# marcemq/crowdmod-ddpm-4D

Hardware: AMD Instinct MI355X
Metric: denoise-steps/sec (UNet fwd + sampler update) at ATC [B,4,T,H,W] (higher is better)
Workload: dtype f32; 1 GPU; config/ATC.yml sampling on the 12x36 grid, fp32 arithmetic (fp32 matrix instructions; fp32 products built from f16 two-way splits -- three v_mfma_f32_32x32x16_f16 cross terms, fp32 accumulate, same error against the reference as round 3's six-term bf16 form -- in the Winograd / quarter-resolution / last-conv layers, whose input is GroupNorm + SiLU output, and in the upsample layers, whose raw inpu; channels=4, past_len=5, future_len=3, global_batch=64, parallelism=batch-shard x1 (2 stream lanes of 32 chains per rank)

## Files before the change

crowdmod-ddpm-4d_amd/csrc/cm_attn_block.hip:

```cpp
#include "cm_kernels.h"

#include <algorithm>
#include <atomic>

namespace cm {

typedef float f32x4 __attribute__((ext_vector_type(4)));

constexpr int ATT_NT = 768;
constexpr int ATT_KS = 3;

template <int D>
__global__ __launch_bounds__(ATT_NT) void attn_head_kernel(const AttnBlockArgs a) {
  constexpr int NT = ATT_NT, NW = NT / 64;
  constexpr int KD = D < 16 ? 16 : D;
  constexpr int DS = KD + 4;
  constexpr int NBQ = (D + 15) / 16;
  constexpr int NBT = 3 * NBQ;
  constexpr int PARTS = D / 8;
  constexpr int E = 4 * D;
  constexpr int XS = E + 8;
  constexpr int Q4 = E >> 2;
  constexpr int RL = NT / Q4;
  extern __shared__ __attribute__((aligned(16))) float sm[];
  const int S = a.S;
  float *Xs = sm;
  float *Wi = Xs + (size_t)S * XS;
  float *Wo = Wi + (size_t)NBT * 16 * XS;
  float *Qs = Wo + (size_t)E * DS;
  float *Ks = Qs + (size_t)S * DS;
  float *Vs = Ks + (size_t)S * DS;
  float *bi = Vs + (size_t)S * DS;
  float *red = bi + NBT * 16;
  const int h = blockIdx.x, b = blockIdx.y, tid = threadIdx.x;
  const int lane = tid & 63, wave = __builtin_amdgcn_readfirstlane(tid >> 6);
  const int r16 = lane & 15, kq = lane >> 4;

  const int q4 = tid % Q4, rl = tid / Q4;
  const float *xb = a.x + (size_t)b * S * E;
  constexpr int UX = 3;
  constexpr int NWI = (NBT * 16 + RL - 1) / RL;
  constexpr int NWO = (E * (KD / 4) + NT - 1) / NT;
  f32x4 vx[UX], vwi[NWI], vwo[NWO];
#pragma unroll
  for (int u = 0; u < UX; ++u) vx[u] = *reinterpret_cast<const f32x4 *>(xb + (size_t)min(rl + u * RL, S - 1) * E + 4 * q4);
#pragma unroll
  for (int u = 0; u < NWI; ++u) {
    const int wr = min(rl + u * RL, NBT * 16 - 1);
    const int which = wr / (NBQ * 16), c = min(wr % (NBQ * 16), D - 1);
    vwi[u] = *reinterpret_cast<const f32x4 *>(a.w_in + (size_t)(which * E + h * D + c) * E + 4 * q4);
  }
#pragma unroll
  for (int u = 0; u < NWO; ++u) {
    const int i = min(tid + u * NT, E * (KD / 4) - 1);
    const int n = i / (KD / 4), c4 = min(i % (KD / 4), D / 4 - 1);
    vwo[u] = *reinterpret_cast<const f32x4 *>(a.w_out + (size_t)n * E + h * D + 4 * c4);
  }
  const f32x4 ga = *reinterpret_cast<const f32x4 *>(a.gamma + 4 * q4);
  const f32x4 be = *reinterpret_cast<const f32x4 *>(a.beta + 4 * q4);
  float bval = 0.f;
  {
    const int tb = min(tid, NBT * 16 - 1);
    const int which = tb / (NBQ * 16), c = min(tb % (NBQ * 16), D - 1);
    bval = a.b_in[which * E + h * D + c];
  }
  float s1 = 0.f;
#pragma unroll
  for (int u = 0; u < UX; ++u) {
    const int row = rl + u * RL;
    if (row < S) {
      *reinterpret_cast<f32x4 *>(Xs + row * XS + 4 * q4) = vx[u];
      s1 += (vx[u][0] + vx[u][1]) + (vx[u][2] + vx[u][3]);
    }
  }
#pragma unroll
  for (int u = 0; u < NWI; ++u) {
    const int wr = rl + u * RL;
    if (wr < NBT * 16) *reinterpret_cast<f32x4 *>(Wi + wr * XS + 4 * q4) = vwi[u];
  }
#pragma unroll
  for (int u = 0; u < NWO; ++u) {
    const int i = tid + u * NT;
    if (i < E * (KD / 4)) {
      const int n = i / (KD / 4), c4 = i % (KD / 4);
      *reinterpret_cast<f32x4 *>(Wo + n * DS + 4 * c4) = (4 * c4 < D) ? vwo[u] : f32x4{0.f, 0.f, 0.f, 0.f};
    }
  }
  if (tid < NBT * 16) bi[tid] = bval;
  for (int row0 = UX * RL; row0 < S; row0 += UX * RL) {
#pragma unroll
    for (int u = 0; u < UX; ++u) vx[u] = *reinterpret_cast<const f32x4 *>(xb + (size_t)min(row0 + rl + u * RL, S - 1) * E + 4 * q4);
#pragma unroll
    for (int u = 0; u < UX; ++u) {
      const int row = row0 + rl + u * RL;
      if (row < S) {
        *reinterpret_cast<f32x4 *>(Xs + row * XS + 4 * q4) = vx[u];
        s1 += (vx[u][0] + vx[u][1]) + (vx[u][2] + vx[u][3]);
      }
    }
  }

  constexpr int QPG = Q4 / 8;
  const int grp = q4 / QPG;
  auto group_sum = [&](float v) -> float {
#pragma unroll
    for (int mk = 1; mk < QPG; mk <<= 1) v += __shfl_xor(v, mk);
    __syncthreads();
    if ((q4 & (QPG - 1)) == 0) red[rl * 8 + grp] = v;
    __syncthreads();
    if (tid < 8) {
      float t = 0.f;
      for (int r = 0; r < RL; ++r) t += red[r * 8 + tid];
      red[RL * 8 + tid] = t;
    }
    __syncthreads();
    return red[RL * 8 + grp];
  };
  const float cnt = (float)(E / 8) * (float)S;
  const float mean = group_sum(s1) / cnt;
  float s2 = 0.f;
  for (int row = rl; row < S; row += RL) {
    const f32x4 v = *reinterpret_cast<const f32x4 *>(Xs + row * XS + 4 * q4);
    const float d0 = v[0] - mean, d1 = v[1] - mean, d2 = v[2] - mean, d3 = v[3] - mean;
    s2 += (d0 * d0 + d1 * d1) + (d2 * d2 + d3 * d3);
  }
  const float rstd = rsqrtf(group_sum(s2) / cnt + a.eps);
  {
    const f32x4 sc = ga * rstd;
    const f32x4 sh = be - sc * mean;
    for (int row = rl; row < S; row += RL) {
      f32x4 *p = reinterpret_cast<f32x4 *>(Xs + row * XS + 4 * q4);
      *p = *p * sc + sh;
    }
  }
  __syncthreads();

  const int nmb = (S + 15) >> 4;
  constexpr int nj = E >> 4;
  const float qscale = rsqrtf((float)D);
  for (int item = wave; item < nmb * NBT; item += NW) {
    const int mb = item / NBT, nb = item - mb * NBT;
    const int arow = min(mb * 16 + r16, S - 1);
    const float *ap = Xs + arow * XS + 4 * kq;
    const float *bp = Wi + (nb * 16 + r16) * XS + 4 * kq;
    f32x4 af[nj], bf[nj];
#pragma unroll
    for (int j = 0; j < nj; ++j) {
      af[j] = *reinterpret_cast<const f32x4 *>(ap + 16 * j);
      bf[j] = *reinterpret_cast<const f32x4 *>(bp + 16 * j);
    }
    f32x4 acc = {0.f, 0.f, 0.f, 0.f};
#pragma unroll
    for (int j = 0; j < nj; ++j)
#pragma unroll
      for (int jj = 0; jj < 4; ++jj) acc = __builtin_amdgcn_mfma_f32_16x16x4f32(af[j][jj], bf[j][jj], acc, 0, 0, 0);
    const int which = nb / NBQ, c = (nb % NBQ) * 16 + r16;
    float *dst = which == 0 ? Qs : (which == 1 ? Ks : Vs);
    const float bias = bi[nb * 16 + r16];
#pragma unroll
    for (int reg = 0; reg < 4; ++reg) {
      const int row = mb * 16 + 4 * kq + reg;
      float v = acc[reg] + bias;
      if (which == 0) v *= qscale;
      if (c >= D) v = 0.f;
      if (row < S) dst[row * DS + c] = v;
    }
  }
  __syncthreads();

  {
    constexpr int LPR = PARTS * ATT_KS;
    constexpr int ROWS = NT / LPR;
    float *mrg = Xs;
    const int part = tid % PARTS, ksl = (tid / PARTS) % ATT_KS, prow = tid / LPR;
    const int kper = (S + ATT_KS - 1) / ATT_KS;
    const int k0 = ksl * kper, k1 = min(S, k0 + kper);
    for (int row0 = 0; row0 < S; row0 += ROWS) {
      const int row = row0 + prow;
      const int rowc = row < S ? row : S - 1;
      const f32x4 q0 = *reinterpret_cast<const f32x4 *>(Qs + rowc * DS + 8 * part);
      const f32x4 q1 = *reinterpret_cast<const f32x4 *>(Qs + rowc * DS + 8 * part + 4);
      f32x4 o0 = {0.f, 0.f, 0.f, 0.f}, o1 = {0.f, 0.f, 0.f, 0.f};
      float mx = -3.0e38f, l = 0.f;
      for (int j = k0; j < k1; ++j) {
        const f32x4 kv0 = *reinterpret_cast<const f32x4 *>(Ks + j * DS + 8 * part);
        const f32x4 kv1 = *reinterpret_cast<const f32x4 *>(Ks + j * DS + 8 * part + 4);
        float sa = q0[0] * kv0[0], sb = q1[0] * kv1[0];
        sa = fmaf(q0[1], kv0[1], sa); sb = fmaf(q1[1], kv1[1], sb);
        sa = fmaf(q0[2], kv0[2], sa); sb = fmaf(q1[2], kv1[2], sb);
        sa = fmaf(q0[3], kv0[3], sa); sb = fmaf(q1[3], kv1[3], sb);
        float sc = sa + sb;
#pragma unroll
        for (int m = 1; m < PARTS; m <<= 1) sc += __shfl_xor(sc, m);
        const f32x4 v0 = *reinterpret_cast<const f32x4 *>(Vs + j * DS + 8 * part);
        const f32x4 v1 = *reinterpret_cast<const f32x4 *>(Vs + j * DS + 8 * part + 4);
        if (sc > mx) {
          const float corr = __expf(mx - sc);
          l *= corr;
          o0 *= corr;
          o1 *= corr;
          mx = sc;
        }
        const float p = __expf(sc - mx);
        l += p;
        o0 += v0 * p;
        o1 += v1 * p;
      }
      __syncthreads();
      if (row < S) {
        float *mp = mrg + ((prow * ATT_KS + ksl) * PARTS + part) * 12;
        mp[0] = mx; mp[1] = l;
        *reinterpret_cast<f32x4 *>(mp + 4) = o0;
        *reinterpret_cast<f32x4 *>(mp + 8) = o1;
      }
      __syncthreads();
      if (ksl == 0 && row < S) {
        float M = -3.0e38f;
#pragma unroll
        for (int s2i = 0; s2i < ATT_KS; ++s2i) M = fmaxf(M, mrg[((prow * ATT_KS + s2i) * PARTS + part) * 12]);
        float L = 0.f;
        f32x4 O0 = {0.f, 0.f, 0.f, 0.f}, O1 = {0.f, 0.f, 0.f, 0.f};
#pragma unroll
        for (int s2i = 0; s2i < ATT_KS; ++s2i) {
          const float *mp = mrg + ((prow * ATT_KS + s2i) * PARTS + part) * 12;
          const float w = (mp[1] > 0.f) ? __expf(mp[0] - M) : 0.f;
          L += mp[1] * w;
          O0 += *reinterpret_cast<const f32x4 *>(mp + 4) * w;
          O1 += *reinterpret_cast<const f32x4 *>(mp + 8) * w;
        }
        const float inv = 1.0f / L;
        *reinterpret_cast<f32x4 *>(Qs + row * DS + 8 * part) = O0 * inv;
        *reinterpret_cast<f32x4 *>(Qs + row * DS + 8 * part + 4) = O1 * inv;
      }
      __syncthreads();
    }
  }

  {
    constexpr int NJ = KD / 16;
    constexpr int nbe = E >> 4;
    float *pout = a.part + ((size_t)h * a.B + b) * (size_t)S * E;
    for (int item = wave; item < nmb * nbe; item += NW) {
      const int mb = item / nbe, nb = item - mb * nbe;
      const int arow = min(mb * 16 + r16, S - 1);
      f32x4 af[NJ], bf[NJ];
#pragma unroll
      for (int j = 0; j < NJ; ++j) {
        af[j] = *reinterpret_cast<const f32x4 *>(Qs + arow * DS + 16 * j + 4 * kq);
        bf[j] = *reinterpret_cast<const f32x4 *>(Wo + (nb * 16 + r16) * DS + 16 * j + 4 * kq);
      }
      f32x4 acc = {0.f, 0.f, 0.f, 0.f};
#pragma unroll
      for (int j = 0; j < NJ; ++j)
#pragma unroll
        for (int jj = 0; jj < 4; ++jj) acc = __builtin_amdgcn_mfma_f32_16x16x4f32(af[j][jj], bf[j][jj], acc, 0, 0, 0);
      const int n = nb * 16 + r16;
#pragma unroll
      for (int reg = 0; reg < 4; ++reg) {
        const int row = mb * 16 + 4 * kq + reg;
        if (row < S) pout[(size_t)row * E + n] = acc[reg];
      }
    }
  }
}

size_t attn_block_lds_bytes(int S, int E, int heads) {
  const int D = E / heads, KD = D < 16 ? 16 : D, NBT = 3 * ((D + 15) / 16);
  return ((size_t)S * (E + 8) + (size_t)NBT * 16 * (E + 8) + (size_t)E * (KD + 4) + (size_t)3 * S * (KD + 4) + (size_t)NBT * 16 +
          (size_t)(ATT_NT / (E / 4)) * 8 + 8) * sizeof(float);
}

bool attn_block_ok(int S, int E, int heads, int groups) {
  if (heads != 4 || E % heads) return false;
  const int D = E / heads;
  if (D != 8 && D != 16 && D != 32) return false;
  if (groups != 8 || E % (4 * groups)) return false;
  return S >= 1 && attn_block_lds_bytes(S, E, heads) <= 160 * 1024;
}

hipError_t launch_attn_block(const AttnBlockArgs &a, hipStream_t st) {
  if (!attn_block_ok(a.S, a.E, a.heads, a.groups)) return hipErrorInvalidValue;
  const int D = a.E / a.heads;
  const size_t smem = attn_block_lds_bytes(a.S, a.E, a.heads);
#define CM_ATTNB(DD)                                                                                        \
  if (D == DD) {                                                                                            \
    static bool attr_set[64] = {false};                                                                     \
    int dev = 0;                                                                                            \
    (void)hipGetDevice(&dev);                                                                               \
    if (!attr_set[dev & 63]) {                                                                              \
      hipError_t e = hipFuncSetAttribute(reinterpret_cast<const void *>(attn_head_kernel<DD>),              \
                                         hipFuncAttributeMaxDynamicSharedMemorySize, 160 * 1024);           \
      if (e != hipSuccess) return e;                                                                        \
      attr_set[dev & 63] = true;                                                                            \
    }                                                                                                       \
    hipLaunchKernelGGL((attn_head_kernel<DD>), dim3(a.heads, a.B), dim3(ATT_NT), smem, st, a);                 \
    return hipGetLastError();                                                                               \
  }
  CM_ATTNB(8) CM_ATTNB(16) CM_ATTNB(32)
#undef CM_ATTNB
  return hipErrorInvalidValue;
}


typedef _Float16 f16x8a __attribute__((ext_vector_type(8)));
typedef unsigned u32x4a __attribute__((ext_vector_type(4)));

constexpr int AS_NT = 1024, AS_E = 128, AS_D = 32, AS_SMAX = 64;
constexpr int AS_HS = AS_E + 8;
constexpr int AS_QS = AS_E + 4;
constexpr int AS_RED = 512;

size_t attn_sample_lds_bytes() {
  return (size_t)2 * AS_SMAX * AS_HS * sizeof(_Float16) + ((size_t)3 * AS_SMAX * AS_QS + AS_RED) * sizeof(float);
}

bool attn_sample_ok(int S, int E, int heads, int groups) { return E == AS_E && heads == 4 && groups == 8 && S >= 1 && S <= AS_SMAX; }

__device__ __forceinline__ float as_range_scale(float m, float *inv) {
  const unsigned e = (__float_as_uint(m) >> 23) & 255u;
  int se = 267 - (int)e;
  se = se < 32 ? 32 : (se > 222 ? 222 : se);
  if (!(m > 0.f) || e == 255u) se = 127;
  *inv = __uint_as_float((unsigned)(254 - se) << 23);
  return __uint_as_float((unsigned)se << 23);
}

__global__ __launch_bounds__(AS_NT) void attn_sample_kernel(const AttnSampleArgs a) {
  constexpr int E = AS_E, D = AS_D, HS = AS_HS, QS = AS_QS, NT = AS_NT;
  extern __shared__ __attribute__((aligned(16))) unsigned char smraw[];
  _Float16 *XH = reinterpret_cast<_Float16 *>(smraw);
  _Float16 *XM = XH + AS_SMAX * HS;
  float *Qs = reinterpret_cast<float *>(XM + AS_SMAX * HS);
  float *Ks = Qs + AS_SMAX * QS;
  float *Vs = Ks + AS_SMAX * QS;
  float *red = Vs + AS_SMAX * QS;
  const int S = a.S, b = blockIdx.x, tid = threadIdx.x;
  const int lane = tid & 63, wave = __builtin_amdgcn_readfirstlane(tid >> 6);
  const int r16 = lane & 15, g4 = lane >> 4;
  const int nrb = (S + 15) >> 4;

  const int q4 = tid & 31, rl = tid >> 5;
  const float *xb = a.x + (size_t)b * S * E;
  f32x4 vx[2];
#pragma unroll
  for (int u = 0; u < 2; ++u) vx[u] = *reinterpret_cast<const f32x4 *>(xb + (size_t)min(rl + 32 * u, S - 1) * E + 4 * q4);
  const f32x4 ga = *reinterpret_cast<const f32x4 *>(a.gamma + 4 * q4);
  const f32x4 be = *reinterpret_cast<const f32x4 *>(a.beta + 4 * q4);
  const int cb0 = 3 * (wave >> 1), rbp = wave & 1;
  const u32x4a *wing = reinterpret_cast<const u32x4a *>(a.win_h2);
  u32x4a wf[3][4][2];
  float bias[3];
#pragma unroll
  for (int ci = 0; ci < 2; ++ci) {
#pragma unroll
    for (int ks = 0; ks < 4; ++ks)
#pragma unroll
      for (int t = 0; t < 2; ++t) wf[ci][ks][t] = wing[(((size_t)(cb0 + ci) * 4 + ks) * 2 + t) * 64 + lane];
  }
#pragma unroll
  for (int ci = 0; ci < 3; ++ci) bias[ci] = a.b_in[(cb0 + ci) * 16 + r16];

  const int grp = q4 >> 2;
  auto group_sum = [&](float v, float *slot) -> float {
    v += __shfl_xor(v, 1);
    v += __shfl_xor(v, 2);
    v += __shfl_xor(v, 32);
    if ((lane & 35) == 0) slot[wave * 8 + grp] = v;
    __syncthreads();
    float t = 0.f;
#pragma unroll
    for (int w = 0; w < NT / 64; ++w) t += slot[w * 8 + grp];
    return t;
  };
  float s1 = 0.f;
#pragma unroll
  for (int u = 0; u < 2; ++u)
    if (rl + 32 * u < S) s1 += (vx[u][0] + vx[u][1]) + (vx[u][2] + vx[u][3]);
  const float cnt = (float)(E / 8) * (float)S;
  const float mean = group_sum(s1, red) / cnt;
  float s2 = 0.f;
#pragma unroll
  for (int u = 0; u < 2; ++u)
    if (rl + 32 * u < S) {
      const float d0 = vx[u][0] - mean, d1 = vx[u][1] - mean, d2 = vx[u][2] - mean, d3 = vx[u][3] - mean;
      s2 += (d0 * d0 + d1 * d1) + (d2 * d2 + d3 * d3);
    }
  const float rstd = rsqrtf(group_sum(s2, red + 128) / cnt + a.eps);

  f32x4 xn[2];
  float amax = 0.f;
  {
    const f32x4 sc = ga * rstd;
    const f32x4 sh = be - sc * mean;
#pragma unroll
    for (int u = 0; u < 2; ++u) {
      xn[u] = vx[u] * sc + sh;
      if (rl + 32 * u < S) amax = fmaxf(amax, fmaxf(fmaxf(fabsf(xn[u][0]), fabsf(xn[u][1])), fmaxf(fabsf(xn[u][2]), fabsf(xn[u][3]))));
      else xn[u] = f32x4{0.f, 0.f, 0.f, 0.f};
    }
  }
  auto sample_max = [&](float v, float *slot) -> float {
#pragma unroll
    for (int off = 32; off >= 1; off >>= 1) v = fmaxf(v, __shfl_xor(v, off));
    if (lane == 0) slot[wave] = v;
    __syncthreads();
    float m = slot[0];
#pragma unroll
    for (int w = 1; w < NT / 64; ++w) m = fmaxf(m, slot[w]);
    return m;
  };
  float isa;
  const float sa = as_range_scale(sample_max(amax, red + 272), &isa);
#pragma unroll
  for (int u = 0; u < 2; ++u) {
    cm_u32x2_t t3[3];
    cm_split2_f16(xn[u] * sa, t3);
    const int row = rl + 32 * u;
    *reinterpret_cast<cm_u32x2_t *>(XH + row * HS + 4 * q4) = t3[0];
    *reinterpret_cast<cm_u32x2_t *>(XM + row * HS + 4 * q4) = t3[1];
  }
  __syncthreads();

  {
    const float osc = a.in_oscale * isa, qscale = rsqrtf((float)D);
#pragma unroll
    for (int ci = 0; ci < 3; ++ci) {
      const int cb = cb0 + ci;
      const int which = cb >> 3, c = (cb & 7) * 16 + r16;
      float *dst = which == 0 ? Qs : (which == 1 ? Ks : Vs);
      for (int rb = rbp; rb < nrb; rb += 2) {
        const _Float16 *ah = XH + (rb * 16 + r16) * HS + 8 * g4, *am = XM + (rb * 16 + r16) * HS + 8 * g4;
        f32x4 acc = {0.f, 0.f, 0.f, 0.f};
#pragma unroll
        for (int ks = 0; ks < 4; ++ks) {
          const f16x8a xh = *reinterpret_cast<const f16x8a *>(ah + 32 * ks), xm = *reinterpret_cast<const f16x8a *>(am + 32 * ks);
          const f16x8a wh = __builtin_bit_cast(f16x8a, wf[ci][ks][0]), wm = __builtin_bit_cast(f16x8a, wf[ci][ks][1]);
          acc = __builtin_amdgcn_mfma_f32_16x16x32_f16(xh, wm, acc, 0, 0, 0);
          acc = __builtin_amdgcn_mfma_f32_16x16x32_f16(xm, wh, acc, 0, 0, 0);
          acc = __builtin_amdgcn_mfma_f32_16x16x32_f16(xh, wh, acc, 0, 0, 0);
        }
#pragma unroll
        for (int reg = 0; reg < 4; ++reg) {
          float v = acc[reg] * osc + bias[ci];
          if (which == 0) v *= qscale;
          dst[(rb * 16 + 4 * g4 + reg) * QS + c] = v;
        }
      }
      if (ci == 0) {
#pragma unroll
        for (int ks = 0; ks < 4; ++ks)
#pragma unroll
          for (int t = 0; t < 2; ++t) wf[2][ks][t] = wing[(((size_t)(cb0 + 2) * 4 + ks) * 2 + t) * 64 + lane];
      }
    }
  }
  const u32x4a *woutg = reinterpret_cast<const u32x4a *>(a.wout_h2);
  const f32x4 bo = *reinterpret_cast<const f32x4 *>(a.b_out + 4 * q4);
#pragma unroll
  for (int u = 0; u < 2; ++u)
    vx[u] = *reinterpret_cast<const f32x4 *>(xb + (size_t)min(rl + 32 * u, S - 1) * E + 4 * q4);
#pragma unroll
  for (int ks = 0; ks < 4; ++ks)
#pragma unroll
    for (int t = 0; t < 2; ++t) wf[0][ks][t] = woutg[(((size_t)(wave >> 1) * 4 + ks) * 2 + t) * 64 + lane];
  __syncthreads();

  const int h = wave >> 2, qb = wave & 3;
  f32x4 oT[2] = {{0.f, 0.f, 0.f, 0.f}, {0.f, 0.f, 0.f, 0.f}};
  float omax = 0.f;
  const bool qvalid = qb * 16 + r16 < S;
  if (qb < nrb) {
    const float *qp = Qs + (qb * 16 + r16) * QS + h * D + 8 * g4;
    const f32x4 q0 = *reinterpret_cast<const f32x4 *>(qp), q1 = *reinterpret_cast<const f32x4 *>(qp + 4);
    f32x4 sc[4];
    float mx = -3.0e38f;
#pragma unroll
    for (int kb = 0; kb < 4; ++kb) {
      sc[kb] = f32x4{-3.0e38f, -3.0e38f, -3.0e38f, -3.0e38f};
      if (kb < nrb) {
        const float *kp = Ks + (kb * 16 + r16) * QS + h * D + 8 * g4;
        const f32x4 k0 = *reinterpret_cast<const f32x4 *>(kp), k1 = *reinterpret_cast<const f32x4 *>(kp + 4);
        f32x4 acc = {0.f, 0.f, 0.f, 0.f};
#pragma unroll
        for (int j = 0; j < 4; ++j) acc = __builtin_amdgcn_mfma_f32_16x16x4f32(k0[j], q0[j], acc, 0, 0, 0);
#pragma unroll
        for (int j = 0; j < 4; ++j) acc = __builtin_amdgcn_mfma_f32_16x16x4f32(k1[j], q1[j], acc, 0, 0, 0);
#pragma unroll
        for (int reg = 0; reg < 4; ++reg) {
          sc[kb][reg] = (kb * 16 + 4 * g4 + reg < S) ? acc[reg] : -3.0e38f;
          mx = fmaxf(mx, sc[kb][reg]);
        }
      }
    }
    mx = fmaxf(mx, __shfl_xor(mx, 16));
    mx = fmaxf(mx, __shfl_xor(mx, 32));
    float l = 0.f;
#pragma unroll
    for (int kb = 0; kb < 4; ++kb)
#pragma unroll
      for (int reg = 0; reg < 4; ++reg) {
        const float p = (kb < nrb && kb * 16 + 4 * g4 + reg < S) ? __expf(sc[kb][reg] - mx) : 0.f;
        sc[kb][reg] = p;
        l += p;
      }
    l += __shfl_xor(l, 16);
    l += __shfl_xor(l, 32);
#pragma unroll
    for (int kb = 0; kb < 4; ++kb)
      if (kb < nrb) {
#pragma unroll
        for (int reg = 0; reg < 4; ++reg) {
          const float *vp = Vs + (kb * 16 + 4 * g4 + reg) * QS + h * D + r16;
          oT[0] = __builtin_amdgcn_mfma_f32_16x16x4f32(vp[0], sc[kb][reg], oT[0], 0, 0, 0);
          oT[1] = __builtin_amdgcn_mfma_f32_16x16x4f32(vp[16], sc[kb][reg], oT[1], 0, 0, 0);
        }
      }
    const float inv = 1.0f / l;
    oT[0] *= inv;
    oT[1] *= inv;
    if (qvalid) {
#pragma unroll
      for (int db = 0; db < 2; ++db)
        omax = fmaxf(omax, fmaxf(fmaxf(fabsf(oT[db][0]), fabsf(oT[db][1])), fmaxf(fabsf(oT[db][2]), fabsf(oT[db][3]))));
    }
  }
  float iso;
  const float so = as_range_scale(sample_max(omax, red + 288), &iso);
  if (qb < nrb) {
#pragma unroll
    for (int db = 0; db < 2; ++db) {
      cm_u32x2_t t3[3];
      cm_split2_f16(qvalid ? oT[db] * so : f32x4{0.f, 0.f, 0.f, 0.f}, t3);
      const int off = (qb * 16 + r16) * HS + h * D + 16 * db + 4 * g4;
      *reinterpret_cast<cm_u32x2_t *>(XH + off) = t3[0];
      *reinterpret_cast<cm_u32x2_t *>(XM + off) = t3[1];
    }
  }
  __syncthreads();

  {
    const float osc = a.out_oscale * iso;
    const int c = (wave >> 1) * 16 + r16;
    for (int rb = rbp; rb < nrb; rb += 2) {
      const _Float16 *ah = XH + (rb * 16 + r16) * HS + 8 * g4, *am = XM + (rb * 16 + r16) * HS + 8 * g4;
      f32x4 acc = {0.f, 0.f, 0.f, 0.f};
#pragma unroll
      for (int ks = 0; ks < 4; ++ks) {
        const f16x8a xh = *reinterpret_cast<const f16x8a *>(ah + 32 * ks), xm = *reinterpret_cast<const f16x8a *>(am + 32 * ks);
        const f16x8a wh = __builtin_bit_cast(f16x8a, wf[0][ks][0]), wm = __builtin_bit_cast(f16x8a, wf[0][ks][1]);
        acc = __builtin_amdgcn_mfma_f32_16x16x32_f16(xh, wm, acc, 0, 0, 0);
        acc = __builtin_amdgcn_mfma_f32_16x16x32_f16(xm, wh, acc, 0, 0, 0);
        acc = __builtin_amdgcn_mfma_f32_16x16x32_f16(xh, wh, acc, 0, 0, 0);
      }
#pragma unroll
      for (int reg = 0; reg < 4; ++reg) Qs[(rb * 16 + 4 * g4 + reg) * QS + c] = acc[reg] * osc;
    }
  }
  __syncthreads();

  float *ob = a.out + (size_t)b * S * E;
#pragma unroll
  for (int u = 0; u < 2; ++u) {
    const int row = rl + 32 * u;
    if (row < S) {
      f32x4 *yp = reinterpret_cast<f32x4 *>(Qs + row * QS + 4 * q4);
      const f32x4 y = (*yp + bo) + vx[u];
      *yp = y;
      *reinterpret_cast<f32x4 *>(ob + (size_t)row * E + 4 * q4) = y;
    }
  }
  if (!a.stat_part) return;
  __syncthreads();
  if (tid < E * a.nslots) {
    const int c = tid & (E - 1), slot = tid >> 7;
    const int r0 = slot * 32, r1 = min(S, r0 + 32);
    float tot = 0.f;
    for (int r = r0; r < r1; ++r) tot += Qs[r * QS + c];
    const float n = (float)(r1 - r0);
    const float mu = tot / n;
    float m2 = 0.f;
    for (int r = r0; r < r1; ++r) { const float d = Qs[r * QS + c] - mu; m2 += d * d; }
    float *sp = a.stat_part + (((size_t)b * a.nslots + slot) * E + c) * 2;
    sp[0] = mu;
    sp[1] = m2;
    if (c == 0) a.stat_cnt[(size_t)b * a.nslots + slot] = n;
  }
}

hipError_t launch_attn_sample(const AttnSampleArgs &a, hipStream_t st) {
  if (!attn_sample_ok(a.S, AS_E, 4, 8) || a.B < 1 || a.nslots != (a.S + 31) / 32 || !a.win_h2 || !a.wout_h2) return hipErrorInvalidValue;
  static std::atomic<bool> attr_set[64];
  int dev = 0;
  (void)hipGetDevice(&dev);
  if (!attr_set[dev & 63].load(std::memory_order_acquire)) {
    hipError_t e = hipFuncSetAttribute(reinterpret_cast<const void *>(attn_sample_kernel), hipFuncAttributeMaxDynamicSharedMemorySize, 160 * 1024);
    if (e != hipSuccess) return e;
    attr_set[dev & 63].store(true, std::memory_order_release);
  }
  hipLaunchKernelGGL(attn_sample_kernel, dim3(a.B), dim3(AS_NT), attn_sample_lds_bytes(), st, a);
  return hipGetLastError();
}

}
```

Before: 978.8 denoise-steps/s, aggregate over 1 GPU under weak scaling (every GPU advances its own batch of 64 chains per step).

## Restructure attention-sample projections: per-wave column pairs, prefetched A fragments, fused epilogue

The QKV input projection now gives 12 waves two column blocks each across all row blocks, instead of 16 waves with three column blocks over half the rows. A shared as_project helper keeps the A fragments in registers and prefetches the next row block, so each fragment load feeds two column blocks of MFMAs. The output projection epilogue writes bias plus residual straight to global memory and LDS in the MFMA layout, which removes one barrier and the row-layout pass. The GroupNorm stat pass is unrolled to 32 register loads with predication. A CM_AS_ABL ablation macro (default 0) is added. In exchange, four waves sit idle during the input projection and the residual loads become scalar strided reads.

```diff
diff --git a/crowdmod-ddpm-4d_amd/csrc/cm_attn_block.hip b/crowdmod-ddpm-4d_amd/csrc/cm_attn_block.hip
--- a/crowdmod-ddpm-4d_amd/csrc/cm_attn_block.hip
+++ b/crowdmod-ddpm-4d_amd/csrc/cm_attn_block.hip
@@ -305,6 +305,10 @@
 typedef _Float16 f16x8a __attribute__((ext_vector_type(8)));
 typedef unsigned u32x4a __attribute__((ext_vector_type(4)));
 
+#ifndef CM_AS_ABL
+#define CM_AS_ABL 0
+#endif
+
 constexpr int AS_NT = 1024, AS_E = 128, AS_D = 32, AS_SMAX = 64;
 constexpr int AS_HS = AS_E + 8;
 constexpr int AS_QS = AS_E + 4;
@@ -323,6 +327,47 @@
   if (!(m > 0.f) || e == 255u) se = 127;
   *inv = __uint_as_float((unsigned)(254 - se) << 23);
   return __uint_as_float((unsigned)se << 23);
+}
+
+template <int NCB, bool ABL, class EP>
+__device__ __forceinline__ void as_project(const _Float16 *XH, const _Float16 *XM, const u32x4a (*wf)[4][2], int rb0, int rbs, int nrb, int r16, int g4, EP &&ep) {
+  if (rb0 >= nrb) return;
+  const int lo = r16 * AS_HS + 8 * g4;
+  f16x8a xa[4][2];
+  auto fetch = [&](int slot, int rb) {
+    const int o = rb * 16 * AS_HS + lo + 32 * slot;
+    xa[slot][0] = *reinterpret_cast<const f16x8a *>(XH + o);
+    xa[slot][1] = *reinterpret_cast<const f16x8a *>(XM + o);
+  };
+  if (!ABL) { fetch(0, rb0); fetch(1, rb0); }
+  for (int rb = rb0; rb < nrb; rb += rbs) {
+    const int rbn = rb + rbs < nrb ? rb + rbs : rb;
+    f32x4 acc[NCB];
+#pragma unroll
+    for (int ci = 0; ci < NCB; ++ci) acc[ci] = f32x4{0.f, 0.f, 0.f, 0.f};
+    if (ABL) {
+#pragma unroll
+      for (int ci = 0; ci < NCB; ++ci) {
+        unsigned k = 0;
+#pragma unroll
+        for (int ks = 0; ks < 4; ++ks) k ^= (wf[ci][ks][0][0] ^ wf[ci][ks][0][3]) ^ (wf[ci][ks][1][0] ^ wf[ci][ks][1][3]);
+        acc[ci][0] = (float)(k & 1u);
+      }
+    }
+#pragma unroll
+    for (int ks = 0; ks < (ABL ? 0 : 4); ++ks) {
+      fetch((ks + 2) & 3, ks < 2 ? rb : rbn);
+      __builtin_amdgcn_sched_barrier(0);
+      const f16x8a xh = xa[ks][0], xm = xa[ks][1];
+#pragma unroll
+      for (int ci = 0; ci < NCB; ++ci) acc[ci] = __builtin_amdgcn_mfma_f32_16x16x32_f16(xh, __builtin_bit_cast(f16x8a, wf[ci][ks][1]), acc[ci], 0, 0, 0);
+#pragma unroll
+      for (int ci = 0; ci < NCB; ++ci) acc[ci] = __builtin_amdgcn_mfma_f32_16x16x32_f16(xm, __builtin_bit_cast(f16x8a, wf[ci][ks][0]), acc[ci], 0, 0, 0);
+#pragma unroll
+      for (int ci = 0; ci < NCB; ++ci) acc[ci] = __builtin_amdgcn_mfma_f32_16x16x32_f16(xh, __builtin_bit_cast(f16x8a, wf[ci][ks][0]), acc[ci], 0, 0, 0);
+    }
+    ep(rb, acc);
+  }
 }
 
 __global__ __launch_bounds__(AS_NT) void attn_sample_kernel(const AttnSampleArgs a) {
@@ -346,19 +391,20 @@
   for (int u = 0; u < 2; ++u) vx[u] = *reinterpret_cast<const f32x4 *>(xb + (size_t)min(rl + 32 * u, S - 1) * E + 4 * q4);
   const f32x4 ga = *reinterpret_cast<const f32x4 *>(a.gamma + 4 * q4);
   const f32x4 be = *reinterpret_cast<const f32x4 *>(a.beta + 4 * q4);
-  const int cb0 = 3 * (wave >> 1), rbp = wave & 1;
+  const bool ipw = wave < 12;
+  const int cb0 = 2 * (ipw ? wave : 0), rbp = wave & 1;
   const u32x4a *wing = reinterpret_cast<const u32x4a *>(a.win_h2);
-  u32x4a wf[3][4][2];
-  float bias[3];
+  u32x4a wf[2][4][2];
+  float bias[2];
 #pragma unroll
   for (int ci = 0; ci < 2; ++ci) {
 #pragma unroll
     for (int ks = 0; ks < 4; ++ks)
 #pragma unroll
-      for (int t = 0; t < 2; ++t) wf[ci][ks][t] = wing[(((size_t)(cb0 + ci) * 4 + ks) * 2 + t) * 64 + lane];
-  }
-#pragma unroll
-  for (int ci = 0; ci < 3; ++ci) bias[ci] = a.b_in[(cb0 + ci) * 16 + r16];
+      for (int t = 0; t < 2; ++t) wf[ci][ks][t] = ipw ? wing[(((size_t)(cb0 + ci) * 4 + ks) * 2 + t) * 64 + lane] : u32x4a{0u, 0u, 0u, 0u};
+  }
+#pragma unroll
+  for (int ci = 0; ci < 2; ++ci) bias[ci] = a.b_in[(cb0 + ci) * 16 + r16];
 
   const int grp = q4 >> 2;
   auto group_sum = [&](float v, float *slot) -> float {
@@ -421,44 +467,29 @@
   }
   __syncthreads();
 
-  {
+  if (ipw) {
     const float osc = a.in_oscale * isa, qscale = rsqrtf((float)D);
-#pragma unroll
-    for (int ci = 0; ci < 3; ++ci) {
-      const int cb = cb0 + ci;
-      const int which = cb >> 3, c = (cb & 7) * 16 + r16;
-      float *dst = which == 0 ? Qs : (which == 1 ? Ks : Vs);
-      for (int rb = rbp; rb < nrb; rb += 2) {
-        const _Float16 *ah = XH + (rb * 16 + r16) * HS + 8 * g4, *am = XM + (rb * 16 + r16) * HS + 8 * g4;
-        f32x4 acc = {0.f, 0.f, 0.f, 0.f};
-#pragma unroll
-        for (int ks = 0; ks < 4; ++ks) {
-          const f16x8a xh = *reinterpret_cast<const f16x8a *>(ah + 32 * ks), xm = *reinterpret_cast<const f16x8a *>(am + 32 * ks);
-          const f16x8a wh = __builtin_bit_cast(f16x8a, wf[ci][ks][0]), wm = __builtin_bit_cast(f16x8a, wf[ci][ks][1]);
-          acc = __builtin_amdgcn_mfma_f32_16x16x32_f16(xh, wm, acc, 0, 0, 0);
-          acc = __builtin_amdgcn_mfma_f32_16x16x32_f16(xm, wh, acc, 0, 0, 0);
-          acc = __builtin_amdgcn_mfma_f32_16x16x32_f16(xh, wh, acc, 0, 0, 0);
+    const int which = cb0 >> 3, c = (cb0 & 7) * 16 + r16;
+    float *dst = which == 0 ? Qs : (which == 1 ? Ks : Vs);
+    as_project<2, (CM_AS_ABL & 2) != 0>(XH, XM, wf, 0, 1, nrb, r16, g4, [&](int rb, const f32x4 *acc) {
+#pragma unroll
+      for (int ci = 0; ci < 2; ++ci)
+#pragma unroll
+        for (int reg = 0; reg < 4; ++reg) {
+          float v = acc[ci][reg] * osc + bias[ci];
+          if (which == 0) v *= qscale;
+          dst[(rb * 16 + 4 * g4 + reg) * QS + c + 16 * ci] = v;
         }
-#pragma unroll
-        for (int reg = 0; reg < 4; ++reg) {
-          float v = acc[reg] * osc + bias[ci];
-          if (which == 0) v *= qscale;
-          dst[(rb * 16 + 4 * g4 + reg) * QS + c] = v;
-        }
-      }
-      if (ci == 0) {
-#pragma unroll
-        for (int ks = 0; ks < 4; ++ks)
-#pragma unroll
-          for (int t = 0; t < 2; ++t) wf[2][ks][t] = wing[(((size_t)(cb0 + 2) * 4 + ks) * 2 + t) * 64 + lane];
-      }
-    }
+    });
   }
   const u32x4a *woutg = reinterpret_cast<const u32x4a *>(a.wout_h2);
-  const f32x4 bo = *reinterpret_cast<const f32x4 *>(a.b_out + 4 * q4);
+  const int oc = (wave >> 1) * 16 + r16;
+  const float bo = a.b_out[oc];
+  float xr[2][4];
 #pragma unroll
   for (int u = 0; u < 2; ++u)
-    vx[u] = *reinterpret_cast<const f32x4 *>(xb + (size_t)min(rl + 32 * u, S - 1) * E + 4 * q4);
+#pragma unroll
+    for (int reg = 0; reg < 4; ++reg) xr[u][reg] = xb[(size_t)min((rbp + 2 * u) * 16 + 4 * g4 + reg, S - 1) * E + oc];
 #pragma unroll
   for (int ks = 0; ks < 4; ++ks)
 #pragma unroll
@@ -469,7 +500,7 @@
   f32x4 oT[2] = {{0.f, 0.f, 0.f, 0.f}, {0.f, 0.f, 0.f, 0.f}};
   float omax = 0.f;
   const bool qvalid = qb * 16 + r16 < S;
-  if (qb < nrb) {
+  if (qb < nrb && !(CM_AS_ABL & 4)) {
     const float *qp = Qs + (qb * 16 + r16) * QS + h * D + 8 * g4;
     const f32x4 q0 = *reinterpret_cast<const f32x4 *>(qp), q1 = *reinterpret_cast<const f32x4 *>(qp + 4);
     f32x4 sc[4];
@@ -540,46 +571,39 @@
 
   {
     const float osc = a.out_oscale * iso;
-    const int c = (wave >> 1) * 16 + r16;
-    for (int rb = rbp; rb < nrb; rb += 2) {
-      const _Float16 *ah = XH + (rb * 16 + r16) * HS + 8 * g4, *am = XM + (rb * 16 + r16) * HS + 8 * g4;
-      f32x4 acc = {0.f, 0.f, 0.f, 0.f};
-#pragma unroll
-      for (int ks = 0; ks < 4; ++ks) {
-        const f16x8a xh = *reinterpret_cast<const f16x8a *>(ah + 32 * ks), xm = *reinterpret_cast<const f16x8a *>(am + 32 * ks);
-        const f16x8a wh = __builtin_bit_cast(f16x8a, wf[0][ks][0]), wm = __builtin_bit_cast(f16x8a, wf[0][ks][1]);
-        acc = __builtin_amdgcn_mfma_f32_16x16x32_f16(xh, wm, acc, 0, 0, 0);
-        acc = __builtin_amdgcn_mfma_f32_16x16x32_f16(xm, wh, acc, 0, 0, 0);
-        acc = __builtin_amdgcn_mfma_f32_16x16x32_f16(xh, wh, acc, 0, 0, 0);
-      }
-#pragma unroll
-      for (int reg = 0; reg < 4; ++reg) Qs[(rb * 16 + 4 * g4 + reg) * QS + c] = acc[reg] * osc;
-    }
-  }
-  __syncthreads();
-
-  float *ob = a.out + (size_t)b * S * E;
-#pragma unroll
-  for (int u = 0; u < 2; ++u) {
-    const int row = rl + 32 * u;
-    if (row < S) {
-      f32x4 *yp = reinterpret_cast<f32x4 *>(Qs + row * QS + 4 * q4);
-      const f32x4 y = (*yp + bo) + vx[u];
-      *yp = y;
-      *reinterpret_cast<f32x4 *>(ob + (size_t)row * E + 4 * q4) = y;
-    }
-  }
+    float *ob = a.out + (size_t)b * S * E;
+    as_project<1, (CM_AS_ABL & 8) != 0>(XH, XM, wf, rbp, 2, nrb, r16, g4, [&](int rb, const f32x4 *acc) {
+#pragma clang fp contract(off)
+#pragma unroll
+      for (int reg = 0; reg < 4; ++reg) {
+        const int row = rb * 16 + 4 * g4 + reg;
+        const float t = acc[0][reg] * osc;
+        const float y = (t + bo) + (rb == rbp ? xr[0][reg] : xr[1][reg]);
+        if (row < S) ob[(size_t)row * E + oc] = y;
+        Qs[row * QS + oc] = y;
+      }
+    });
+  }
+
   if (!a.stat_part) return;
   __syncthreads();
   if (tid < E * a.nslots) {
     const int c = tid & (E - 1), slot = tid >> 7;
-    const int r0 = slot * 32, r1 = min(S, r0 + 32);
+    const int r0 = slot * 32, nr = min(S, r0 + 32) - r0;
+    constexpr int NR = (CM_AS_ABL & 1) ? 1 : 32;
+    const float *col = Qs + r0 * QS + c;
+    float yv[NR];
+#pragma unroll
+    for (int i = 0; i < NR; ++i) yv[i] = col[i * QS];
+    __builtin_amdgcn_sched_barrier(0);
     float tot = 0.f;
-    for (int r = r0; r < r1; ++r) tot += Qs[r * QS + c];
-    const float n = (float)(r1 - r0);
+#pragma unroll
+    for (int i = 0; i < NR; ++i) { const float t = tot + yv[i]; tot = i < nr ? t : tot; }
+    const float n = (float)nr;
     const float mu = tot / n;
     float m2 = 0.f;
-    for (int r = r0; r < r1; ++r) { const float d = Qs[r * QS + c] - mu; m2 += d * d; }
+#pragma unroll
+    for (int i = 0; i < NR; ++i) { const float d = yv[i] - mu, t = fmaf(d, d, m2); m2 = i < nr ? t : m2; }
     float *sp = a.stat_part + (((size_t)b * a.nslots + slot) * E + c) * 2;
     sp[0] = mu;
     sp[1] = m2;
```

Measured after the change: 984.5 denoise-steps/s, aggregate over 1 GPU under weak scaling (every GPU advances its own batch of 64 chains per step), median of 6. Within noise of the previous version (+0.6%).
